# Lennart0HU/Master-Thesis-Deep-Reinforcement-Learning-DDPG-in-Home-Energy-Management

Hardware: AMD Instinct MI355X
Metric: env-steps/sec (higher is better)
Workload: dtype f32; 1 GPU; 65536 parallel shems_LU1 envs per GPU, Charger98 synthetic train table (4320 rows), 72-step episodes, mode=train; envs_per_gpu=65536, episode_len=72, mode=train

## Files before the change

master-thesis-deep-reinforcement-learning-ddpg-in-home-energy-management_amd/_build.py:

```python
from __future__ import annotations

import os
import shutil
import subprocess

HERE = os.path.dirname(os.path.abspath(__file__))
CSRC = os.path.join(HERE, "csrc")
ROOT = os.path.dirname(HERE)
LIB = os.path.join(HERE, "libshems_hip.so")
ARCH = "gfx950"

UNITS = [
    ("shems_capi.hip", []),
    ("shems_env.hip", ["-ffp-contract=off"]),
    ("shems_policy.hip", []),
    ("shems_ddpg.hip", []),
    ("shems_gupd.hip", []),
    ("shems_track.hip", ["-ffp-contract=off"]),
    ("shems_foresight.hip", ["-ffp-contract=off"]),
    ("shems_wide.hip", []),
    ("shems_train.hip", []),
    ("shems_dp.hip", []),
]
COMMON = ["-O3", "-fPIC", "-std=c++17", f"--offload-arch={ARCH}", "-Wall", "-Wno-unused-function", "-Wno-unused-value", "-Wno-unused-result",
          "-I" + os.path.join(ROOT, "include")]


def _hipcc():
    for cand in (os.environ.get("HIPCC"), shutil.which("hipcc"), "/opt/rocm/bin/hipcc"):
        if cand and os.path.exists(cand):
            return cand
    raise RuntimeError("hipcc not found: libshems_hip.so cannot be built (there is no CPU fallback)")


def _deps(src):
    d = [src]
    for f in os.listdir(CSRC):
        if f.endswith(".h"):
            d.append(os.path.join(CSRC, f))
    d.append(os.path.join(ROOT, "include", "shems_hip.h"))
    d.append(os.path.abspath(__file__))
    return d


def build(force=False, verbose=False, defines=(), tag=""):
    hipcc = _hipcc()
    objs = []
    rebuilt = False
    outdir = HERE if not tag else os.path.join(ROOT, "build")
    objdir = CSRC if not tag else outdir
    os.makedirs(outdir, exist_ok=True)
    lib = os.path.join(outdir, f"libshems_hip{tag}.so")
    for name, extra in UNITS:
        src = os.path.join(CSRC, name)
        if not os.path.exists(src):
            continue
        extra = list(extra) + ["-D" + d for d in defines]
        obj = os.path.join(objdir, name.rsplit(".", 1)[0] + tag + ".o")
        stale = force or not os.path.exists(obj) or any(os.path.getmtime(p) > os.path.getmtime(obj) for p in _deps(src))
        if stale:
            cmd = [hipcc, *COMMON, *extra, "-c", src, "-o", obj]
            if verbose:
                print(" ".join(cmd), flush=True)
            subprocess.check_call(cmd)
            rebuilt = True
        objs.append(obj)
    if rebuilt or not os.path.exists(lib):
        cmd = [hipcc, "-shared", "-fPIC", f"--offload-arch={ARCH}", "-o", lib, *objs, "-ldl"]
        if verbose:
            print(" ".join(cmd), flush=True)
        subprocess.check_call(cmd)
    return lib


if __name__ == "__main__":
    import sys
    if "--stamp-act" in sys.argv:
        print(build(force="--force" in sys.argv, verbose=True, defines=("SHEMS_STAMP_ACT",), tag="_stampact"))
    elif "--stamp" in sys.argv:
        print(build(force="--force" in sys.argv, verbose=True, defines=("SHEMS_STAMP",), tag="_stamp"))
    else:
        print(build(force="--force" in sys.argv, verbose=True))
```

master-thesis-deep-reinforcement-learning-ddpg-in-home-energy-management_amd/csrc/shems_policy.hip:

```cpp
#include <hip/hip_runtime.h>

#include <cstdlib>
#include <cstdio>
#include <cstring>
#include <type_traits>

#include "shems_env_dev.h"
#include "shems_internal.h"

namespace shems {

typedef float f32x16 __attribute__((ext_vector_type(16)));
typedef float f32x4 __attribute__((ext_vector_type(4)));
typedef float f32x2 __attribute__((ext_vector_type(2)));
template <int N> struct FVec { typedef float type __attribute__((ext_vector_type(N))); };
template <> struct FVec<1> { typedef float type; };
template <int N> __device__ __forceinline__ float fvec_get(const typename FVec<N>::type &v, int i) { return v[i]; }
template <> __device__ __forceinline__ float fvec_get<1>(const float &v, int) { return v; }

constexpr int kIn = 9, kH1 = SHEMS_L1, kH2 = SHEMS_L2, kOut = 2;

template <int NA> __device__ __forceinline__ int act_col(int nbase, int t, int row) { return nbase + 64 * (t >> 1) + 2 * row + (t & 1); }
template <int NA> __device__ __forceinline__ typename FVec<NA>::type act_load_a(const float *row_at_nbase, int li);
template <> __device__ __forceinline__ FVec<4>::type act_load_a<4>(const float *p, int li)
{
    const f32x2 x = *reinterpret_cast<const f32x2 *>(p + 2 * li), y = *reinterpret_cast<const f32x2 *>(p + 64 + 2 * li);
    return FVec<4>::type{x[0], x[1], y[0], y[1]};
}
constexpr int kKC = 16;
constexpr int kChunks = 16;
constexpr int kW1K = 10, kW1C = 256;
constexpr int kOffB1 = kIn * kH1, kOffW2 = kOffB1 + kH1, kOffB2 = kOffW2 + kH1 * kH2, kOffW3 = kOffB2 + kH2,
              kOffB3 = kOffW3 + kH2 * kOut;
static_assert(kOffB3 + kOut == SHEMS_ACTOR_PARAMS, "actor layout");
static_assert(kW1K == 10 && kIn == 9, "L1_TILE's MFMA chain is written out for 5 k-steps: 9 inputs + the bias row");
constexpr int kH2P = 512;
constexpr int kTailFloats = kH2P + kH2P * kOut + kOut;

struct ActArgs {
    shems_view v;
    shems_act_params p;
    const float *obs;
    int64_t m;
    int64_t m0;
    float *a_out;
    double *rewards;
    float *rewards_f32;
    double *block_reward;
    double *returns_acc;
    shems_replay ring;
    shems_ring_window win;
    int do_step;
    int use_ring;
    int gcount;
    int64_t gstride;
    int64_t genvs;
    const float *w2t;
    int tm_max;
};

template <class T>
__device__ __forceinline__ T *gsh(T *p, int64_t off)
{
    typedef typename std::conditional<std::is_const<T>::value, const char, char>::type B;
    return p ? reinterpret_cast<T *>(reinterpret_cast<B *>(p) + off) : p;
}

constexpr int kFreeChunkFloats = kKC * 128;
constexpr int kPreDw = 16;
constexpr int act_h_rows(int tm) { return tm == 4 ? 128 : 256; }
constexpr bool act_tail_pre(int tm) { return tm <= 2; }
template <int TM, int NW, int RD>
constexpr size_t act_lds_bytes()
{
    return sizeof(float) * ((NW * RD * kFreeChunkFloats + 16) + act_h_rows(TM) * 32 * TM + kW1K * 32 * TM + kW1K * kW1C +
                            (kTailFloats + 2) + 32 * TM * kIn + (act_tail_pre(TM) ? 32 * TM * kPreDw : 0));
}

__device__ __forceinline__ uint32_t lds_addr(const void *p)
{
    return (uint32_t)(uintptr_t)(const __attribute__((address_space(3))) void *)p;
}
template <int IMM>
__device__ __forceinline__ void glds16_asm(const char *sbase, uint32_t voff, uint32_t lds_base)
{
    asm volatile("s_mov_b32 m0, %2\n\ts_nop 0\n\tglobal_load_lds_dwordx4 %0, %1 offset:%3"
                 :: "v"(voff), "s"(sbase), "s"(lds_base), "i"(IMM) : "memory");
}

__device__ __forceinline__ void glds16_asm_piece8(const char *sbase, uint32_t voff, uint32_t lds_base, int q)
{
    switch (q) {
    case 0: glds16_asm<-4096>(sbase, voff, lds_base); break;
    case 1: glds16_asm<-3072>(sbase, voff, lds_base); break;
    case 2: glds16_asm<-2048>(sbase, voff, lds_base); break;
    case 3: glds16_asm<-1024>(sbase, voff, lds_base); break;
    case 4: glds16_asm<0>(sbase, voff, lds_base); break;
    case 5: glds16_asm<1024>(sbase, voff, lds_base); break;
    case 6: glds16_asm<2048>(sbase, voff, lds_base); break;
    default: glds16_asm<3072>(sbase, voff, lds_base); break;
    }
}

__device__ __forceinline__ float2 gauss_pair(uint64_t seed, uint32_t tick, int64_t i)
{
    const u32x4 x = philox4x32_10((uint32_t)i, (uint32_t)((uint64_t)i >> 32), tick, kStreamNoise, (uint32_t)seed,
                                  (uint32_t)(seed >> 32));
    const float u1 = ((float)(x.x >> 8) + 1.0f) * (1.0f / 16777216.0f);
    const float u2 = u01_24(x.y);
    const float r = sqrtf(-2.0f * logf(u1));
    float s, c;
    sincosf(6.28318530717958647692f * u2, &s, &c);
    return make_float2(r * c, r * s);
}

#ifdef SHEMS_STAMP_ACT
#define PSTAMP(i) do { if (threadIdx.x == 0 && blockIdx.x == 0) { reinterpret_cast<unsigned long long *>(A.block_reward)[2*(i)] = __builtin_amdgcn_s_memtime(); reinterpret_cast<unsigned long long *>(A.block_reward)[2*(i)+1] = __builtin_amdgcn_s_memrealtime(); } } while (0)
#else
#define PSTAMP(i)
#endif
#ifdef SHEMS_STAMP_ACT
#define TSTAMP(i) do { asm volatile("s_waitcnt vmcnt(0) lgkmcnt(0)" ::: "memory"); PSTAMP(i); } while (0)
#else
#define TSTAMP(i)
#endif

struct NoiseDraw { uint32_t a, b, c; };
__device__ __forceinline__ NoiseDraw noise_draw(const shems_act_params &p, int64_t i)
{
    NoiseDraw d = {0u, 0u, 0u};
    if (!p.train) return d;
    if (p.noise_kind == SHEMS_NOISE_EPS) {
        const u32x4 x = philox4x32_10((uint32_t)i, (uint32_t)((uint64_t)i >> 32), p.tick, kStreamNoise, (uint32_t)p.seed, (uint32_t)(p.seed >> 32));
        d.a = x.x; d.b = x.y; d.c = x.z;
    } else {
        const float2 z = gauss_pair(p.seed, p.tick, i);
        d.a = __float_as_uint(z.x); d.b = __float_as_uint(z.y);
    }
    return d;
}

struct TailPre {
    Row nx;
    float h_cur;
    int32_t idx, step, ci;
    NoiseDraw nz;
};
__device__ __forceinline__ void tailpre_store(float *lds, const TailPre &t)
{
    f32x4 *q = reinterpret_cast<f32x4 *>(lds);
    q[0] = f32x4{t.nx.h, t.nx.soc_ev, t.nx.d_e, t.nx.g_e};
    q[1] = f32x4{t.nx.p_buy, t.nx.h_cos, t.nx.h_sin, t.nx.season};
    q[2] = f32x4{t.h_cur, __int_as_float(t.idx), __int_as_float(t.step), __int_as_float(t.ci)};
    q[3] = f32x4{__uint_as_float(t.nz.a), __uint_as_float(t.nz.b), __uint_as_float(t.nz.c), 0.0f};
// ... 723 lines not shown
    typedef typename FVec<TM>::type BVec;
    f32x16 acc[2][TM];
#pragma unroll
    for (int a = 0; a < 2; ++a)
#pragma unroll
        for (int r = 0; r < 16; ++r) {
            const float bias = tl[act_col<2>(nbase, a, (r & 3) + 8 * (r >> 2) + 4 * lh)];
#pragma unroll
            for (int b = 0; b < TM; ++b) acc[a][b][r] = bias;
        }
    constexpr int kGKsteps = (kChunks - 1) * (kKC / 2) + (kH1 - (kChunks - 1) * kKC) / 2;
    f32x2 af_[3];
    BVec bf_[3];
#define G_KSTEP(c, ks)                                                                                          \
    do {                                                                                                        \
        const int K_ = 8 * (c) + (ks), K2_ = K_ + 2;                                                            \
        if (K2_ < kGKsteps) {                                                                                   \
            const int c2_ = K2_ >> 3, kr_ = 2 * (K2_ & 7) + lh;                                                 \
            af_[K2_ % 3] = *reinterpret_cast<const f32x2 *>(Wg + (c2_ % RD) * kGChunkFloats + kr_ * 64 + 2 * li); \
            bf_[K2_ % 3] = *reinterpret_cast<const BVec *>(Hc + (c2_ * kKC + kr_) * BM + TM * li);              \
        }                                                                                                       \
        _Pragma("unroll") for (int b = 0; b < TM; ++b)                                                          \
            acc[0][b] = __builtin_amdgcn_mfma_f32_32x32x2f32(af_[K_ % 3][0], fvec_get<TM>(bf_[K_ % 3], b), acc[0][b], 0, 0, 0); \
        _Pragma("unroll") for (int b = 0; b < TM; ++b)                                                          \
            acc[1][b] = __builtin_amdgcn_mfma_f32_32x32x2f32(af_[K_ % 3][1], fvec_get<TM>(bf_[K_ % 3], b), acc[1][b], 0, 0, 0); \
        __builtin_amdgcn_sched_group_barrier(0x008, TM, 0);                                                     \
        __builtin_amdgcn_sched_group_barrier(0x100, 1, 0);                                                      \
        __builtin_amdgcn_sched_group_barrier(0x008, TM, 0);                                                     \
        __builtin_amdgcn_sched_group_barrier(0x100, 1, 0);                                                      \
        __builtin_amdgcn_sched_barrier(0);                                                                      \
        if ((ks) < g_pieces((c) + RD - 1)) { G_PIECE((c) + RD - 1, (ks) < kGPieces ? (ks) : 0); __builtin_amdgcn_sched_barrier(0); } \
    } while (0)
#define G_CHUNK(c, NKS)                                                                                         \
    do {                                                                                                        \
        _Pragma("unroll") for (int ks = 0; ks < ((NKS) < 6 ? (NKS) : 6); ++ks) G_KSTEP(c, ks);                  \
        if ((c) + 1 < kChunks) {                                                                                \
            constexpr int keep_ = g_keep<RD>(c);                                                                \
            asm volatile("s_waitcnt vmcnt(%0)" ::"n"(keep_) : "memory");       \
            __builtin_amdgcn_sched_barrier(0);                                                                  \
        }                                                                                                       \
        _Pragma("unroll") for (int ks = 6; ks < (NKS); ++ks) G_KSTEP(c, ks);                                    \
    } while (0)
    {
        constexpr int keep0_ = g_keep<RD>(-1);
        asm volatile("s_waitcnt vmcnt(%0)" ::"n"(keep0_) : "memory");
        __builtin_amdgcn_sched_barrier(0);
    }
#ifdef SHEMS_STAMP_ACT
    if (lane == 0 && blockIdx.x == 0) reinterpret_cast<unsigned long long *>(A.block_reward)[48 + wave] = __builtin_amdgcn_s_memtime();
#endif
#pragma unroll
    for (int k0 = 0; k0 < 2; ++k0) {
        af_[k0] = *reinterpret_cast<const f32x2 *>(Wg + (2 * k0 + lh) * 64 + 2 * li);
        bf_[k0] = *reinterpret_cast<const BVec *>(Hc + (2 * k0 + lh) * BM + TM * li);
    }
    __builtin_amdgcn_sched_barrier(0);
    G_CHUNK(0, kKC / 2);  GSTAMP(3, blockIdx.x == 0); G_CHUNK(1, kKC / 2);  G_CHUNK(2, kKC / 2);  G_CHUNK(3, kKC / 2);
    G_CHUNK(4, kKC / 2);  G_CHUNK(5, kKC / 2);  G_CHUNK(6, kKC / 2);  G_CHUNK(7, kKC / 2);
    G_CHUNK(8, kKC / 2);  G_CHUNK(9, kKC / 2);  G_CHUNK(10, kKC / 2); G_CHUNK(11, kKC / 2);
    G_CHUNK(12, kKC / 2); G_CHUNK(13, kKC / 2); G_CHUNK(14, kKC / 2);
    GSTAMP(4, blockIdx.x == 0);
    G_CHUNK(15, (kH1 - (kChunks - 1) * kKC) / 2);

    GSTAMP(10, blockIdx.x == 0);
#ifdef SHEMS_STAMP_ACT
    if (lane == 0 && blockIdx.x == 0) reinterpret_cast<unsigned long long *>(A.block_reward)[32 + wave] = __builtin_amdgcn_s_memtime();
#endif
    {
        const float *w3s = tl + kH2P;
        float u0[TM], u1[TM];
#pragma unroll
        for (int t = 0; t < 2; ++t) {
            float o0[TM], o1[TM];
#pragma unroll
            for (int b = 0; b < TM; ++b) { o0[b] = 0.0f; o1[b] = 0.0f; }
#pragma unroll
            for (int r = 0; r < 16; ++r) {
                const int n = act_col<2>(nbase, t, (r & 3) + 8 * (r >> 2) + 4 * lh);
                const float2 w3 = *reinterpret_cast<const float2 *>(w3s + 2 * n);
#pragma unroll
                for (int b = 0; b < TM; ++b) {
                    const float h = fmaxf(acc[t][b][r], 0.0f);
                    o0[b] = fmaf(h, w3.x, o0[b]);
                    o1[b] = fmaf(h, w3.y, o1[b]);
                }
            }
#pragma unroll
            for (int b = 0; b < TM; ++b) {
                u0[b] = t == 0 ? o0[b] : u0[b] + o0[b];
                u1[b] = t == 0 ? o1[b] : u1[b] + o1[b];
            }
        }
#pragma unroll
        for (int b = 0; b < TM; ++b) {
            const float g0 = u0[b] + __shfl_xor(u0[b], 32, 64), g1 = u1[b] + __shfl_xor(u1[b], 32, 64);
            if (lh == 0) *reinterpret_cast<float2 *>(red + (g * BM + TM * li + b) * 2) = make_float2(g0, g1);
        }
    }
    __syncthreads();
    GSTAMP(8, blockIdx.x == 0);

    double reward = 0.0;
    const int64_t i = env0 + tid;
    bool fin = tid < BM && i < A.m;
    float p0 = 0.0f, p1 = 0.0f;
    if (fin) {
        auto half_sum = [&](int hf, int j) {
            return ((red[((4 * hf) * BM + tid) * 2 + j] + red[((4 * hf + 1) * BM + tid) * 2 + j]) + red[((4 * hf + 2) * BM + tid) * 2 + j]) +
                   red[((4 * hf + 3) * BM + tid) * 2 + j];
        };
        float h00, h01, h10, h11;
        if constexpr (NS == 1) {
            h00 = half_sum(0, 0); h01 = half_sum(0, 1); h10 = half_sum(1, 0); h11 = half_sum(1, 1);
        } else {
            float m0 = half_sum(half, 0), m1 = half_sum(half, 1);
            unsigned long long mine = ((unsigned long long)__float_as_uint(m1) << 32) | __float_as_uint(m0);
            if (mine == kSplitEmpty) { mine = 0x7FC000007FC00000ull; m0 = m1 = __uint_as_float(0x7FC00000u); }
            unsigned long long *slot = X.slot + tile * BM + tid;
            const unsigned long long got = __hip_atomic_exchange(slot, mine, __ATOMIC_RELAXED, __HIP_MEMORY_SCOPE_AGENT);
            if (got == kSplitEmpty) fin = false;
            else __hip_atomic_store(slot, kSplitEmpty, __ATOMIC_RELAXED, __HIP_MEMORY_SCOPE_AGENT);
            const float o0 = __uint_as_float((uint32_t)got), o1 = __uint_as_float((uint32_t)(got >> 32));
            h00 = half == 0 ? m0 : o0; h01 = half == 0 ? m1 : o1;
            h10 = half == 0 ? o0 : m0; h11 = half == 0 ? o1 : m1;
        }
        p0 = tl[kH2P + kH2P * kOut + 0] + (h00 + h10);
        p1 = tl[kH2P + kH2P * kOut + 1] + (h01 + h11);
    }
    GSTAMP(9, blockIdx.x == 0);
    GSTAMP(11, tile == 0 && fin);
    if (fin) reward = act_env_tail<HP>(A, i, p0, p1, learner, goff, A.obs == A.v.obs ? xR + tid * kIn : nullptr, xP + tid * kPreDw, hp, gx);
    GSTAMP(12, tile == 0 && fin);
#ifndef SHEMS_STAMP_ACT
    if (NS == 1 && A.block_reward) {
        __syncthreads();
        double *red64 = reinterpret_cast<double *>(Wc);
        const double s = block_sum(reward, red64, NW);
        if (tid == 0) A.block_reward[tile] = s;
    }
#endif
}
template <int TM, int NW, int NS, int RD>
__global__ __launch_bounds__(64 * NW) void k_actg(ActArgs A, ActSplit X) { k_actg_body<TM, NW, NS, RD, 0>(A, X, nullptr); }
template <int TM, int NW, int NS, int RD>
__global__ __launch_bounds__(64 * NW) void k_actg_hp(ActArgs A, ActSplit X, const shems_group_hparams *hp) { k_actg_body<TM, NW, NS, RD, 1>(A, X, hp); }
template <int TM, int NW, int NS, int RD>
__global__ __launch_bounds__(64 * NW) void k_actg_x(ActArgs A, ActSplit X, const shems_group_hparams *hp, GroupX gx) { k_actg_body<TM, NW, NS, RD, 2>(A, X, hp, gx); }

constexpr int k2CR = 4, k2RD = 4, k2CF = k2CR * 128;
constexpr int k2NCH = (kH1 + k2CR - 1) / k2CR;
constexpr int k2_pieces(int ch) { return ch < 0 || ch >= k2NCH ? 0 : ch == k2NCH - 1 ? (kH1 - (k2NCH - 1) * k2CR + 1) / 2 : k2CR / 2; }
constexpr size_t act2_lds_bytes()
{
    return sizeof(float) * (4 * k2RD * k2CF + 16 + 128 * 64 + kW1K * 64 + (kTailFloats + 2) + 64 * kPreDw + 4);
}

__device__ __forceinline__ void k2_piece(const char *sbase, uint32_t voff, uint32_t lds_base, int q)
{
    if (q == 0) glds16_asm<-1024>(sbase, voff, lds_base); else glds16_asm<0>(sbase, voff, lds_base);
}

template <int HP>
__device__ __forceinline__ void k_act2_body(const ActArgs &A, const shems_group_hparams *hp, const GroupX gx = GroupX{nullptr, nullptr})
{
    constexpr int TM = 2, BM = 64, NA = 4, NT_ = 256, HR = 128;
    extern __shared__ __attribute__((aligned(16))) char smem[];
    float *Wc = reinterpret_cast<float *>(smem);
    float *Hc = Wc + 4 * k2RD * k2CF + 16;
    float *xT = Hc + HR * BM;
    float *tl = xT + kW1K * BM;
    float *xP = tl + (kTailFloats + 2);
    const int tid = threadIdx.x;
    const int lane = tid & 63, wave = __builtin_amdgcn_readfirstlane(tid >> 6);
    const int li = lane & 31, lh = lane >> 5;
    int64_t bid = blockIdx.x;
    if (A.gcount > 1 && (gridDim.x & 7) == 0) bid = (int64_t)(blockIdx.x & 7) * (gridDim.x >> 3) + (blockIdx.x >> 3);
    const int64_t env0 = A.m0 + bid * BM;
    const int64_t learner = A.gcount > 1 ? env0 / A.genvs : 0;
    const int64_t goff = learner * A.gstride;
    const float *__restrict__ P = gsh(A.p.actor, goff);
    const float *__restrict__ s_min = gsh(A.p.s_min, goff), *__restrict__ s_max = gsh(A.p.s_max, goff);
    const int nbase = 128 * wave;

    const char *W2g = reinterpret_cast<const char *>(P + kOffW2);
    float *Wf = Wc + wave * (k2RD * k2CF);
    const uint32_t ring_lds = lds_addr(Wf) + 1024;
    const char *wsbase = W2g + wave * 512;
    uint32_t wvoff[2];
#pragma unroll
    for (int q = 0; q < 2; ++q) wvoff[q] = (uint32_t)((lane >> 5) * (kH2 * 4) + (lane & 31) * 16 + q * (2 * kH2 * 4) - (q - 1) * 1024);
#define K2_PIECE(chunk, q) k2_piece(wsbase + (size_t)(chunk) * (k2CR * kH2 * 4), wvoff[q], ring_lds + ((chunk) % k2RD) * (k2CF * 4), (q))
    TailPre tp;
    const bool view = A.do_step != 0, multi = view && A.v.n_cfg > 1;
    {
        const int64_t pe = min(env0 + (tid & (BM - 1)), A.m - 1);
        const int32_t *pidx = view ? A.v.idx : reinterpret_cast<const int32_t *>(P), *pstep = view ? A.v.step : reinterpret_cast<const int32_t *>(P);
        const uint16_t *pci = multi ? A.v.cfg_of_env : reinterpret_cast<const uint16_t *>(P);
        tp.idx = pidx[view ? pe : 0];
        tp.ci = multi ? (int)pci[pe] : 0;
        tp.step = pstep[view ? pe : 0];
    }
    constexpr int kIt = (BM * kIn + NT_ - 1) / NT_;
    float sv[kIt], lo[kIt], hi[kIt], tv[6];
    const int64_t last = A.m * kIn - 1;
#pragma unroll
    for (int it = 0; it < kIt; ++it) {
        const int e = min(it * NT_ + tid, BM * kIn - 1), k = e % kIn;
        sv[it] = A.obs[min(env0 * kIn + e, last)];
        lo[it] = s_min[k];
        hi[it] = s_max[k];
    }
#pragma unroll
    for (int it = 0; it < 6; ++it) tv[it] = P[kOffB2 + min(it * 256 + tid, kH2 + kH2 * kOut + kOut - 1)];
#define K2_L1_LOAD(gbase, a0_, a1_, kA_, kB_)                                                     \
    _Pragma("unroll") for (int s_ = 0; s_ < kW1K / 2; ++s_) {                                     \
        const int j_ = 2 * s_ + lh;                                                               \
        a0_[s_] = P[j_ * kH1 + min(kA_, kH1 - 1)];                                                \
        a1_[s_] = P[j_ * kH1 + min(kB_, kH1 - 1)];                                                \
    }
    const int t0 = wave, t1 = wave + 4;
    const int kA0 = 32 * (t0 >> 1) + li, kB0 = 32 * (t1 >> 1) + li;
    float wa0[kW1K / 2], wb0[kW1K / 2];
    K2_L1_LOAD(0, wa0, wb0, kA0, kB0)
    tp.nz = noise_draw(A.p, env0 + (tid & (BM - 1)));
    f32x4 ra, rb;
    {
        const int32_t *pc = view ? reinterpret_cast<const int32_t *>(A.v.cfgs + tp.ci) : reinterpret_cast<const int32_t *>(P);
        constexpr int o_row0 = offsetof(shems_config, table_row0) / 4, o_nrow = offsetof(shems_config, nrow) / 4;
        const int32_t row0 = pc[o_row0], nrow = pc[o_nrow];
        const float *tp_tables = view ? A.v.tables : P;
        const int64_t tp_row = view ? (int64_t)row0 + max(min(tp.idx + 1, nrow), 2) - 1 : 1;
        const f32x4 *rp = reinterpret_cast<const f32x4 *>(tp_tables + tp_row * SHEMS_NCOL);
        ra = rp[0]; rb = rp[1];
        tp.h_cur = tp_tables[(tp_row - 1) * SHEMS_NCOL];
    }
#pragma unroll
    for (int it = 0; it < kIt; ++it) {
        const int e = it * NT_ + tid, m = e / kIn, k = e - m * kIn;
        const float x = (sv[it] - lo[it]) / ((hi[it] - lo[it]) + 1e-8f);
        if (e < BM * kIn) xT[k * BM + m] = env0 * kIn + e <= last ? x : 0.0f;
    }
    if (tid < BM) xT[kIn * BM + tid] = 1.0f;
    {
#pragma unroll
        for (int it = 0; it < 6; ++it) {
            const int e = it * 256 + tid;
            if (e < kH2) tl[e] = tv[it];
            else if (e < kH2 + kH2 * kOut) tl[kH2P + (e - kH2)] = tv[it];
            else if (e < kH2 + kH2 * kOut + kOut) tl[kH2P + kH2P * kOut + (e - kH2 - kH2 * kOut)] = tv[it];
        }
        if (tid < kH2P - kH2) tl[kH2 + tid] = 0.0f;
        if (tid < (kH2P - kH2) * kOut) tl[kH2P + kH2 * kOut + tid] = 0.0f;
    }
    asm volatile("s_waitcnt lgkmcnt(0)\n\ts_barrier" ::: "memory");
#pragma unroll
    for (int ch = 0; ch < k2RD - 1; ++ch)
#pragma unroll
        for (int q = 0; q < 2; ++q) K2_PIECE(ch, q);

#define K2_L1_PHASE(gbase, a0_, a1_)                                                              \
    do {                                                                                          \
        const int gA_ = (gbase) + (t0 >> 1), bA_ = t0 & 1, gB_ = (gbase) + (t1 >> 1), bB_ = t1 & 1; \
        float c0_[kW1K / 2], c1_[kW1K / 2], z0_[kW1K / 2], z1_[kW1K / 2];                         \
        _Pragma("unroll") for (int s_ = 0; s_ < kW1K / 2; ++s_) {                                 \
            const int j_ = 2 * s_ + lh;                                                           \
            c0_[s_] = xT[j_ * BM + TM * li + bA_];                                                \
            c1_[s_] = xT[j_ * BM + TM * li + bB_];                                                \
            z0_[s_] = 32 * gA_ + li < kH1 ? a0_[s_] : 0.0f;                                       \
            z1_[s_] = 32 * gB_ + li < kH1 ? a1_[s_] : 0.0f;                                       \
        }                                                                                         \
        f32x16 u0_, u1_;                                                                          \
        asm volatile("s_nop 1\n\t"                                                                \
                     "v_mfma_f32_32x32x2_f32 %0, %2, %7, 0\n\t"                                   \
                     "v_mfma_f32_32x32x2_f32 %1, %12, %17, 0\n\t"                                 \
                     "v_mfma_f32_32x32x2_f32 %0, %3, %8, %0\n\t"                                  \
                     "v_mfma_f32_32x32x2_f32 %1, %13, %18, %1\n\t"                                \
                     "v_mfma_f32_32x32x2_f32 %0, %4, %9, %0\n\t"                                  \
                     "v_mfma_f32_32x32x2_f32 %1, %14, %19, %1\n\t"                                \
                     "v_mfma_f32_32x32x2_f32 %0, %5, %10, %0\n\t"                                 \
                     "v_mfma_f32_32x32x2_f32 %1, %15, %20, %1\n\t"                                \
                     "v_mfma_f32_32x32x2_f32 %0, %6, %11, %0\n\t"                                 \
                     "v_mfma_f32_32x32x2_f32 %1, %16, %21, %1\n\t"                                \
                     "s_nop 15\n\ts_nop 7"                                                        \
                     : "=&v"(u0_), "=&v"(u1_)                                                     \
                     : "v"(z0_[0]), "v"(z0_[1]), "v"(z0_[2]), "v"(z0_[3]), "v"(z0_[4]),           \
                       "v"(c0_[0]), "v"(c0_[1]), "v"(c0_[2]), "v"(c0_[3]), "v"(c0_[4]),           \
                       "v"(z1_[0]), "v"(z1_[1]), "v"(z1_[2]), "v"(z1_[3]), "v"(z1_[4]),           \
                       "v"(c1_[0]), "v"(c1_[1]), "v"(c1_[2]), "v"(c1_[3]), "v"(c1_[4]));          \
        float *d0_ = Hc + ((gA_ * 32) % HR) * BM + TM * li + bA_, *d1_ = Hc + ((gB_ * 32) % HR) * BM + TM * li + bB_; \
        _Pragma("unroll") for (int r_ = 0; r_ < 16; ++r_) {                                       \
            d0_[((r_ & 3) + 8 * (r_ >> 2) + 4 * lh) * BM] = fmaxf(u0_[r_], 0.0f);                 \
            d1_[((r_ & 3) + 8 * (r_ >> 2) + 4 * lh) * BM] = fmaxf(u1_[r_], 0.0f);                 \
        }                                                                                         \
    } while (0)
    K2_L1_PHASE(0, wa0, wb0);
    float wa1[kW1K / 2], wb1[kW1K / 2];
    {
        const int kA1 = 128 + kA0, kB1 = 128 + kB0;
        K2_L1_LOAD(4, wa1, wb1, kA1, kB1)
    }
    tp.nx = Row{ra[0], ra[1], ra[2], ra[3], rb[0], rb[1], rb[2], rb[3]};
    tailpre_store(xP + (tid & (BM - 1)) * kPreDw, tp);
    asm volatile("s_waitcnt lgkmcnt(0)\n\ts_barrier" ::: "memory");

    typedef FVec<NA>::type AVec;
    typedef FVec<TM>::type BVec;
    f32x16 acc[NA][TM];
#pragma unroll
    for (int a = 0; a < NA; ++a)
#pragma unroll
        for (int r = 0; r < 16; ++r) {
            const float bias = tl[act_col<NA>(nbase, a, (r & 3) + 8 * (r >> 2) + 4 * lh)];
#pragma unroll
            for (int b = 0; b < TM; ++b) acc[a][b][r] = bias;
        }
    constexpr int kKsteps = kH1 / 2;
    AVec af_[3];
    BVec bf_[3];
#define K2_KSTEP(K)                                                                                             \
    do {                                                                                                        \
        constexpr int K2_ = (K) + 2, c2_ = K2_ >> 1, klim_ = (K) < 64 ? 64 : kKsteps;                           \
        if (K2_ < klim_) {                                                                                      \
            if ((K2_ & 1) == 0) {                                                                               \
                asm volatile("s_waitcnt vmcnt(%0)" ::"n"(k2_pieces(c2_ + 1)) : "memory");                       \
                __builtin_amdgcn_sched_barrier(0);                                                              \
            }                                                                                                   \
            const int kr_ = 2 * (K2_ & 1) + lh;                                                                 \
            af_[K2_ % 3] = act_load_a<NA>(Wf + (c2_ % k2RD) * k2CF + kr_ * 128, li);                            \
            bf_[K2_ % 3] = *reinterpret_cast<const BVec *>(Hc + ((2 * K2_) % HR + lh) * BM + TM * li);          \
        }                                                                                                       \
        _Pragma("unroll") for (int a = 0; a < NA; ++a)                                                          \
            _Pragma("unroll") for (int b = 0; b < TM; ++b)                                                      \
                acc[a][b] = __builtin_amdgcn_mfma_f32_32x32x2f32(fvec_get<NA>(af_[(K) % 3], a), fvec_get<TM>(bf_[(K) % 3], b), acc[a][b], 0, 0, 0); \
        __builtin_amdgcn_sched_group_barrier(0x008, 2, 0);                                                      \
        __builtin_amdgcn_sched_group_barrier(0x100, 1, 0);                                                      \
        __builtin_amdgcn_sched_group_barrier(0x008, 2, 0);                                                      \
        __builtin_amdgcn_sched_group_barrier(0x100, 1, 0);                                                      \
        __builtin_amdgcn_sched_barrier(0);                                                                      \
        if (((K) & 1) < k2_pieces(((K) >> 1) + k2RD - 1)) { K2_PIECE(((K) >> 1) + k2RD - 1, (K) & 1); __builtin_amdgcn_sched_barrier(0); } \
    } while (0)
#define K2_K4(K) K2_KSTEP(K); K2_KSTEP((K) + 1); K2_KSTEP((K) + 2); K2_KSTEP((K) + 3)
#define K2_K16(K) K2_K4(K); K2_K4((K) + 4); K2_K4((K) + 8); K2_K4((K) + 12)
    asm volatile("s_waitcnt vmcnt(%0)" ::"n"(k2_pieces(1) + k2_pieces(2)) : "memory");
    __builtin_amdgcn_sched_barrier(0);
#pragma unroll
    for (int k0 = 0; k0 < 2; ++k0) {
        af_[k0] = act_load_a<NA>(Wf + (2 * k0 + lh) * 128, li);
        bf_[k0] = *reinterpret_cast<const BVec *>(Hc + (2 * k0 + lh) * BM + TM * li);
    }
    __builtin_amdgcn_sched_barrier(0);
    K2_K16(0); K2_K16(16); K2_K16(32); K2_K16(48);
    asm volatile("s_waitcnt lgkmcnt(0)\n\ts_barrier" ::: "memory");
    K2_L1_PHASE(4, wa1, wb1);
    asm volatile("s_waitcnt lgkmcnt(0)\n\ts_barrier" ::: "memory");
    asm volatile("s_waitcnt vmcnt(%0)" ::"n"(k2_pieces(33) + k2_pieces(34)) : "memory");
    __builtin_amdgcn_sched_barrier(0);
#pragma unroll
    for (int k0 = 0; k0 < 2; ++k0) {
        af_[(64 + k0) % 3] = act_load_a<NA>(Wf + ((32 + (k0 >> 1)) % k2RD) * k2CF + (2 * (k0 & 1) + lh) * 128, li);
        bf_[(64 + k0) % 3] = *reinterpret_cast<const BVec *>(Hc + (2 * k0 + lh) * BM + TM * li);
    }
    __builtin_amdgcn_sched_barrier(0);
    K2_K16(64); K2_K16(80); K2_K16(96); K2_K4(112); K2_K4(116); K2_K4(120); K2_KSTEP(124);

    const float *w3s = tl + kH2P;
#pragma unroll
    for (int gl = 0; gl < 2; ++gl) {
        float u0[TM], u1[TM];
#pragma unroll
        for (int t = 0; t < 2; ++t) {
            const int a = 2 * gl + t;
            float o0[TM], o1[TM];
#pragma unroll
            for (int b = 0; b < TM; ++b) { o0[b] = 0.0f; o1[b] = 0.0f; }
#pragma unroll
            for (int r = 0; r < 16; ++r) {
                const int n = act_col<NA>(nbase, a, (r & 3) + 8 * (r >> 2) + 4 * lh);
                const float2 w3 = *reinterpret_cast<const float2 *>(w3s + 2 * n);
#pragma unroll
                for (int b = 0; b < TM; ++b) {
                    const float h = fmaxf(acc[a][b][r], 0.0f);
                    o0[b] = fmaf(h, w3.x, o0[b]);
                    o1[b] = fmaf(h, w3.y, o1[b]);
                }
            }
#pragma unroll
            for (int b = 0; b < TM; ++b) {
                u0[b] = t == 0 ? o0[b] : u0[b] + o0[b];
                u1[b] = t == 0 ? o1[b] : u1[b] + o1[b];
            }
        }
#pragma unroll
        for (int b = 0; b < TM; ++b) {
            const float g0 = u0[b] + __shfl_xor(u0[b], 32, 64), g1 = u1[b] + __shfl_xor(u1[b], 32, 64);
            if (lh == 0) *reinterpret_cast<float2 *>(Wf + gl * (BM * kOut) + (TM * li + b) * 2) = make_float2(g0, g1);
        }
    }
    __syncthreads();
    double reward = 0.0;
    const int64_t i = env0 + tid;
    if (tid < BM && i < A.m) {
        float hs[2][2];
#pragma unroll
        for (int hf = 0; hf < 2; ++hf)
#pragma unroll
            for (int j = 0; j < 2; ++j) {
                const float *r0 = Wc + (2 * hf) * (k2RD * k2CF), *r1 = Wc + (2 * hf + 1) * (k2RD * k2CF);
                hs[hf][j] = ((r0[tid * 2 + j] + r0[BM * kOut + tid * 2 + j]) + r1[tid * 2 + j]) + r1[BM * kOut + tid * 2 + j];
            }
        const float p0 = tl[kH2P + kH2P * kOut + 0] + (hs[0][0] + hs[1][0]), p1 = tl[kH2P + kH2P * kOut + 1] + (hs[0][1] + hs[1][1]);
        reward = act_env_tail<HP>(A, i, p0, p1, learner, goff, nullptr, xP + tid * kPreDw, hp, gx);
    }
#ifndef SHEMS_STAMP_ACT
    if (A.block_reward) {
        __syncthreads();
        double *red64 = reinterpret_cast<double *>(Hc);
        const double s = block_sum(reward, red64, 4);
        if (tid == 0) A.block_reward[bid] = s;
    }
#endif
}
__global__ __launch_bounds__(256, 2) void k_act2(ActArgs A) { k_act2_body<0>(A, nullptr); }
__global__ __launch_bounds__(256, 2) void k_act2_hp(ActArgs A, const shems_group_hparams *hp) { k_act2_body<1>(A, hp); }
__global__ __launch_bounds__(256, 2) void k_act2_x(ActArgs A, const shems_group_hparams *hp, GroupX gx) { k_act2_body<2>(A, hp, gx); }

static int launch_act2(const ActArgs &a, hipStream_t st, const shems_group_hparams *hp = nullptr, const GroupX *gx = nullptr)
{
    constexpr size_t lds = act2_lds_bytes();
    static_assert(lds <= 80 * 1024, "k_act2: two workgroups must fit a CU's 160 KB");
    static std::atomic<uint64_t> optin{0}, optin_hp{0}, optin_x{0};
    const dim3 grid((unsigned)((a.m - a.m0 + 63) / 64));
    if (gx) {
        if (int rc = lds_optin(optin_x, reinterpret_cast<const void *>(&k_act2_x), (int)lds, "hipFuncSetAttribute(k_act2_x)")) return rc;
        hipLaunchKernelGGL(k_act2_x, grid, dim3(256), lds, st, a, hp, *gx);
        return hip_ok(hipGetLastError(), "k_act2_x launch");
    }
    if (hp) {
        if (int rc = lds_optin(optin_hp, reinterpret_cast<const void *>(&k_act2_hp), (int)lds, "hipFuncSetAttribute(k_act2_hp)")) return rc;
        hipLaunchKernelGGL(k_act2_hp, grid, dim3(256), lds, st, a, hp);
        return hip_ok(hipGetLastError(), "k_act2_hp launch");
    }
    if (int rc = lds_optin(optin, reinterpret_cast<const void *>(&k_act2), (int)lds, "hipFuncSetAttribute(k_act2)")) return rc;
    hipLaunchKernelGGL(k_act2, grid, dim3(256), lds, st, a);
    return hip_ok(hipGetLastError(), "k_act2 launch");
}

static int pick_tm(int64_t m, int tm_max = 0)
{
    const int tm = m >= 256 * 128 ? 4 : m >= 256 * 64 ? 2 : 1;
    return tm_max > 0 && tm > tm_max ? tm_max : tm;
}
static int group_tm_max(int64_t envs_per_learner) { return envs_per_learner % 128 == 0 ? 4 : envs_per_learner % 64 == 0 ? 2 : 1; }

template <int TM, int NW, int RD>
static int launch_act(const ActArgs &a, hipStream_t st, const shems_group_hparams *hp = nullptr, const GroupX *gx = nullptr)
{
    constexpr int BM = 32 * TM;
    const size_t lds = act_lds_bytes<TM, NW, RD>();
    static_assert(act_lds_bytes<TM, NW, RD>() <= 160 * 1024, "k_act: LDS image exceeds 160 KB");
    static std::atomic<uint64_t> optin{0}, optin_hp{0}, optin_x{0};
    const unsigned grid = (unsigned)((a.m - a.m0 + BM - 1) / BM);
    if (gx) {
        if (int rc = lds_optin(optin_x, reinterpret_cast<const void *>(&k_act_x<TM, NW, RD>), (int)lds, "hipFuncSetAttribute(k_act_x)")) return rc;
        hipLaunchKernelGGL((k_act_x<TM, NW, RD>), dim3(grid), dim3(64 * NW), lds, st, a, hp, *gx);
        return hip_ok(hipGetLastError(), "k_act_x launch");
    }
    if (hp) {
        if (int rc = lds_optin(optin_hp, reinterpret_cast<const void *>(&k_act_hp<TM, NW, RD>), (int)lds, "hipFuncSetAttribute(k_act_hp)")) return rc;
        hipLaunchKernelGGL((k_act_hp<TM, NW, RD>), dim3(grid), dim3(64 * NW), lds, st, a, hp);
        return hip_ok(hipGetLastError(), "k_act_hp launch");
    }
    if (int rc = lds_optin(optin, reinterpret_cast<const void *>(&k_act<TM, NW, RD>), (int)lds, "hipFuncSetAttribute(k_act)")) return rc;
    hipLaunchKernelGGL((k_act<TM, NW, RD>), dim3(grid), dim3(64 * NW), lds, st, a);
    return hip_ok(hipGetLastError(), "k_act launch");
}

constexpr int kSplitMaxTiles = 512;
static int split_scratch(hipStream_t st, ActSplit *out)
{
    struct Slot { int dev; hipStream_t st; ActSplit x; };
    static Slot slots[32];
    static int nslots = 0;
    static std::atomic_flag lock = ATOMIC_FLAG_INIT;
    int dev = 0;
    if (int rc = hip_ok(hipGetDevice(&dev), "hipGetDevice")) return rc;
    while (lock.test_and_set(std::memory_order_acquire)) {}
    int rc = SHEMS_OK;
    int found = -1;
    for (int i = 0; i < nslots; ++i)
        if (slots[i].dev == dev && slots[i].st == st) { found = i; break; }
    if (found < 0) {
        if (nslots == 32) rc = set_error(SHEMS_ERR_ARG, "k_actg: more than 32 (device, stream) pairs use the column-split form");
        else {
            ActSplit x = {nullptr};
            const size_t bytes = (size_t)kSplitMaxTiles * 64 * sizeof(unsigned long long);
            rc = hip_ok(hipMalloc((void **)&x.slot, bytes), "hipMalloc(split slots)");
            if (!rc) rc = hip_ok(hipMemset(x.slot, 0xFF, bytes), "hipMemset(split slots)");
            if (!rc) { slots[nslots] = Slot{dev, st, x}; found = nslots++; }
        }
    }
    if (!rc) *out = slots[found].x;
    lock.clear(std::memory_order_release);
    return rc;
}

template <int TM, int NW, int NS, int RD>
static int launch_actg(const ActArgs &a, hipStream_t st, const shems_group_hparams *hp = nullptr, const GroupX *gx = nullptr)
{
    constexpr int BM = 32 * TM;
    constexpr size_t lds = actg_lds_bytes<TM, NW, RD>();
    static_assert(lds <= 160 * 1024, "k_actg: LDS image exceeds 160 KB");
    static std::atomic<uint64_t> optin{0}, optin_hp{0}, optin_x{0};
    if (gx) {
        if (int rc = lds_optin(optin_x, reinterpret_cast<const void *>(&k_actg_x<TM, NW, NS, RD>), (int)lds, "hipFuncSetAttribute(k_actg_x)")) return rc;
    } else if (hp) {
        if (int rc = lds_optin(optin_hp, reinterpret_cast<const void *>(&k_actg_hp<TM, NW, NS, RD>), (int)lds, "hipFuncSetAttribute(k_actg_hp)")) return rc;
    } else if (int rc = lds_optin(optin, reinterpret_cast<const void *>(&k_actg<TM, NW, NS, RD>), (int)lds, "hipFuncSetAttribute(k_actg)")) return rc;
    const int64_t tiles = (a.m - a.m0 + BM - 1) / BM;
    ActSplit x = {nullptr};
    if constexpr (NS == 2) {
        if (tiles > kSplitMaxTiles) return set_error(SHEMS_ERR_ARG, "k_actg: %lld env tiles exceed the split form's scratch", (long long)tiles);
        if (split_scratch(st, &x) != SHEMS_OK) {
            return launch_actg<1, 8, 1, RD>(a, st, hp, gx);
        }
    }
    if (gx) {
        hipLaunchKernelGGL((k_actg_x<TM, NW, NS, RD>), dim3((unsigned)(tiles * NS)), dim3(64 * NW), lds, st, a, x, hp, *gx);
        return hip_ok(hipGetLastError(), "k_actg_x launch");
    }
    if (hp) {
        hipLaunchKernelGGL((k_actg_hp<TM, NW, NS, RD>), dim3((unsigned)(tiles * NS)), dim3(64 * NW), lds, st, a, x, hp);
        return hip_ok(hipGetLastError(), "k_actg_hp launch");
    }
    hipLaunchKernelGGL((k_actg<TM, NW, NS, RD>), dim3((unsigned)(tiles * NS)), dim3(64 * NW), lds, st, a, x);
    return hip_ok(hipGetLastError(), "k_actg launch");
}

static int act_form() { static const int f = []() { const char *e = getenv("SHEMS_ACT_FORM"); return e ? atoi(e) : -1; }(); return f; }
enum ActForm { kAct2, kAct442, kAct242, kAct142, kAct143, kActg1422, kActg1423, kActg1813 };
static const char *act_form_name(ActForm f)
{
    static const char *const names[] = {"shems::k_act2", "shems::k_act<4, 4, 2>", "shems::k_act<2, 4, 2>", "shems::k_act<1, 4, 2>",
                                        "shems::k_act<1, 4, 3>", "shems::k_actg<1, 4, 2, 2>", "shems::k_actg<1, 4, 2, 3>",
                                        "shems::k_actg<1, 8, 1, 3>"};
    return names[f];
}
static int act_form_tile_envs(ActForm f)
{
    switch (f) {
    case kAct2: return 64;
    case kAct442: return 128;
    case kAct242: return 64;
    default: return 32;
    }
}

static ActForm pick_act_form(int64_t cnt, int tm_max, int gcount, bool w2t, bool want_sum)
{
    const int form = act_form();
    if (w2t) {
        const int tmt = pick_tm(cnt, tm_max);
        return tmt == 4 ? kAct442 : tmt == 2 ? kAct242 : kAct142;
    }
    if (form < 0 && cnt > 8192 && gcount <= 1) return kAct2;
    if (form == 12 && (tm_max == 0 || tm_max >= 2)) return kAct2;
    const int tm = pick_tm(cnt, tm_max);
    if (tm == 4) return kAct442;
    if (tm == 2) return kAct242;
    if (form == 2) return kAct142;
    if (form == 3) return kAct143;
    const bool split_fits = (cnt + 31) / 32 <= kSplitMaxTiles;
    if ((form == 10 || (form < 0 && cnt > 128 * 32)) && !want_sum && split_fits) return kActg1422;
    if (form == 8 || !split_fits || (form != 9 && (cnt > 128 * 32 || want_sum))) return kActg1813;
    return kActg1423;
}

static int act_tile_envs(int64_t m) { return act_form_tile_envs(pick_act_form(m, 0, 0, false, true)); }

static int dispatch_act(const ActArgs &a, hipStream_t st, const shems_group_hparams *hp = nullptr, const GroupX *gx = nullptr)
{
#ifdef SHEMS_STAMP_ACT
    const bool want_sum = false;
#else
    const bool want_sum = a.block_reward != nullptr;
// ... 298 lines not shown
```

Baseline: 397.5 million env-steps/s.

## Make k_act2 persistent and prefetch next tile's inputs and weights

Turns the actor+env kernel into a persistent loop with a grid capped at two workgroups per CU. Each workgroup walks its tiles and prefetches the next tile's observations, indices, table rows and the first W2 ring chunks plus L1 weights while finishing the current tile's tail. The aim is to hide per-tile prologue latency and cut block launch overhead. It adds register pressure and LDS for normalization bounds, uses compiler-barrier tricks and a disable-machine-licm flag to curb hoisting, and risks load imbalance or spills.

```diff
diff --git a/master-thesis-deep-reinforcement-learning-ddpg-in-home-energy-management_amd/_build.py b/master-thesis-deep-reinforcement-learning-ddpg-in-home-energy-management_amd/_build.py
--- a/master-thesis-deep-reinforcement-learning-ddpg-in-home-energy-management_amd/_build.py
+++ b/master-thesis-deep-reinforcement-learning-ddpg-in-home-energy-management_amd/_build.py
@@ -13,7 +13,7 @@
 UNITS = [
     ("shems_capi.hip", []),
     ("shems_env.hip", ["-ffp-contract=off"]),
-    ("shems_policy.hip", []),
+    ("shems_policy.hip", ["-mllvm", "-disable-machine-licm"]),
     ("shems_ddpg.hip", []),
     ("shems_gupd.hip", []),
     ("shems_track.hip", ["-ffp-contract=off"]),
diff --git a/master-thesis-deep-reinforcement-learning-ddpg-in-home-energy-management_amd/csrc/shems_policy.hip b/master-thesis-deep-reinforcement-learning-ddpg-in-home-energy-management_amd/csrc/shems_policy.hip
--- a/master-thesis-deep-reinforcement-learning-ddpg-in-home-energy-management_amd/csrc/shems_policy.hip
+++ b/master-thesis-deep-reinforcement-learning-ddpg-in-home-energy-management_amd/csrc/shems_policy.hip
@@ -1,5 +1,6 @@
 #include <hip/hip_runtime.h>
 
+#include <algorithm>
 #include <cstdlib>
 #include <cstdio>
 #include <cstring>
@@ -1029,13 +1030,21 @@
 constexpr int k2_pieces(int ch) { return ch < 0 || ch >= k2NCH ? 0 : ch == k2NCH - 1 ? (kH1 - (k2NCH - 1) * k2CR + 1) / 2 : k2CR / 2; }
 constexpr size_t act2_lds_bytes()
 {
-    return sizeof(float) * (4 * k2RD * k2CF + 16 + 128 * 64 + kW1K * 64 + (kTailFloats + 2) + 64 * kPreDw + 4);
+    return sizeof(float) * (4 * k2RD * k2CF + 16 + 128 * 64 + kW1K * 64 + (kTailFloats + 2) + 64 * kPreDw + 32 + 4);
 }
 
 __device__ __forceinline__ void k2_piece(const char *sbase, uint32_t voff, uint32_t lds_base, int q)
 {
     if (q == 0) glds16_asm<-1024>(sbase, voff, lds_base); else glds16_asm<0>(sbase, voff, lds_base);
 }
+
+__device__ __forceinline__ const ActArgs &k2_args_again()
+{
+    uint32_t z = 0;
+    asm volatile("" : "+s"(z));
+    return *(const ActArgs *)((const __attribute__((address_space(4))) char *)__builtin_amdgcn_kernarg_segment_ptr() + z);
+}
+__device__ __forceinline__ int k2_again(int x) { asm volatile("" : "+v"(x)); return x; }
 
 template <int HP>
 __device__ __forceinline__ void k_act2_body(const ActArgs &A, const shems_group_hparams *hp, const GroupX gx = GroupX{nullptr, nullptr})
@@ -1047,12 +1056,14 @@
     float *xT = Hc + HR * BM;
     float *tl = xT + kW1K * BM;
     float *xP = tl + (kTailFloats + 2);
-    const int tid = threadIdx.x;
+    float *nb = xP + BM * kPreDw;
+    const int tid = threadIdx.x, tid0 = tid;
     const int lane = tid & 63, wave = __builtin_amdgcn_readfirstlane(tid >> 6);
     const int li = lane & 31, lh = lane >> 5;
-    int64_t bid = blockIdx.x;
-    if (A.gcount > 1 && (gridDim.x & 7) == 0) bid = (int64_t)(blockIdx.x & 7) * (gridDim.x >> 3) + (blockIdx.x >> 3);
-    const int64_t env0 = A.m0 + bid * BM;
+    const int64_t ntiles = (A.m - A.m0 + BM - 1) / BM;
+    int64_t tile = blockIdx.x;
+    if (A.gcount > 1 && (gridDim.x & 7) == 0) tile = (int64_t)(blockIdx.x & 7) * (gridDim.x >> 3) + (blockIdx.x >> 3);
+    int64_t env0 = A.m0 + tile * BM;
     const int64_t learner = A.gcount > 1 ? env0 / A.genvs : 0;
     const int64_t goff = learner * A.gstride;
     const float *__restrict__ P = gsh(A.p.actor, goff);
@@ -1066,42 +1077,29 @@
     uint32_t wvoff[2];
 #pragma unroll
     for (int q = 0; q < 2; ++q) wvoff[q] = (uint32_t)((lane >> 5) * (kH2 * 4) + (lane & 31) * 16 + q * (2 * kH2 * 4) - (q - 1) * 1024);
-#define K2_PIECE(chunk, q) k2_piece(wsbase + (size_t)(chunk) * (k2CR * kH2 * 4), wvoff[q], ring_lds + ((chunk) % k2RD) * (k2CF * 4), (q))
-    TailPre tp;
+    const char *wst = wsbase;
+    const float *__restrict__ Pt = P;
+#define K2_PIECE(chunk, q) k2_piece(wst + (size_t)(chunk) * (k2CR * kH2 * 4), wvoff[q], ring_lds + ((chunk) % k2RD) * (k2CF * 4), (q))
+#define K2_RING_START()                                                                           \
+    _Pragma("unroll") for (int ch_ = 0; ch_ < k2RD - 1; ++ch_)                                    \
+        _Pragma("unroll") for (int q_ = 0; q_ < 2; ++q_) K2_PIECE(ch_, q_)
+    K2_RING_START();
     const bool view = A.do_step != 0, multi = view && A.v.n_cfg > 1;
-    {
-        const int64_t pe = min(env0 + (tid & (BM - 1)), A.m - 1);
+    constexpr int kIt = (BM * kIn + NT_ - 1) / NT_;
+    const int64_t last = A.m * kIn - 1;
+    struct TileIn { float sv[kIt]; int32_t idx, step, ci; };
+    auto tile_in = [&](const ActArgs &A, int tid, int64_t e0, TileIn &t) {
+        const int64_t pe = min(e0 + (tid & (BM - 1)), A.m - 1);
         const int32_t *pidx = view ? A.v.idx : reinterpret_cast<const int32_t *>(P), *pstep = view ? A.v.step : reinterpret_cast<const int32_t *>(P);
         const uint16_t *pci = multi ? A.v.cfg_of_env : reinterpret_cast<const uint16_t *>(P);
-        tp.idx = pidx[view ? pe : 0];
-        tp.ci = multi ? (int)pci[pe] : 0;
-        tp.step = pstep[view ? pe : 0];
-    }
-    constexpr int kIt = (BM * kIn + NT_ - 1) / NT_;
-    float sv[kIt], lo[kIt], hi[kIt], tv[6];
-    const int64_t last = A.m * kIn - 1;
-#pragma unroll
-    for (int it = 0; it < kIt; ++it) {
-        const int e = min(it * NT_ + tid, BM * kIn - 1), k = e % kIn;
-        sv[it] = A.obs[min(env0 * kIn + e, last)];
-        lo[it] = s_min[k];
-        hi[it] = s_max[k];
-    }
-#pragma unroll
-    for (int it = 0; it < 6; ++it) tv[it] = P[kOffB2 + min(it * 256 + tid, kH2 + kH2 * kOut + kOut - 1)];
-#define K2_L1_LOAD(gbase, a0_, a1_, kA_, kB_)                                                     \
-    _Pragma("unroll") for (int s_ = 0; s_ < kW1K / 2; ++s_) {                                     \
-        const int j_ = 2 * s_ + lh;                                                               \
-        a0_[s_] = P[j_ * kH1 + min(kA_, kH1 - 1)];                                                \
-        a1_[s_] = P[j_ * kH1 + min(kB_, kH1 - 1)];                                                \
-    }
-    const int t0 = wave, t1 = wave + 4;
-    const int kA0 = 32 * (t0 >> 1) + li, kB0 = 32 * (t1 >> 1) + li;
-    float wa0[kW1K / 2], wb0[kW1K / 2];
-    K2_L1_LOAD(0, wa0, wb0, kA0, kB0)
-    tp.nz = noise_draw(A.p, env0 + (tid & (BM - 1)));
-    f32x4 ra, rb;
-    {
+        t.idx = pidx[view ? pe : 0];
+        t.ci = multi ? (int)pci[pe] : 0;
+        t.step = pstep[view ? pe : 0];
+#pragma unroll
+        for (int it = 0; it < kIt; ++it) t.sv[it] = A.obs[min(e0 * kIn + min(it * NT_ + tid, BM * kIn - 1), last)];
+    };
+    auto tile_pre = [&](const ActArgs &A, int tid, int64_t e0, const TileIn &t, TailPre &tp, f32x4 &ra, f32x4 &rb) {
+        tp.idx = t.idx; tp.ci = t.ci; tp.step = t.step;
         const int32_t *pc = view ? reinterpret_cast<const int32_t *>(A.v.cfgs + tp.ci) : reinterpret_cast<const int32_t *>(P);
         constexpr int o_row0 = offsetof(shems_config, table_row0) / 4, o_nrow = offsetof(shems_config, nrow) / 4;
         const int32_t row0 = pc[o_row0], nrow = pc[o_nrow];
@@ -1110,14 +1108,27 @@
         const f32x4 *rp = reinterpret_cast<const f32x4 *>(tp_tables + tp_row * SHEMS_NCOL);
         ra = rp[0]; rb = rp[1];
         tp.h_cur = tp_tables[(tp_row - 1) * SHEMS_NCOL];
-    }
-#pragma unroll
-    for (int it = 0; it < kIt; ++it) {
-        const int e = it * NT_ + tid, m = e / kIn, k = e - m * kIn;
-        const float x = (sv[it] - lo[it]) / ((hi[it] - lo[it]) + 1e-8f);
-        if (e < BM * kIn) xT[k * BM + m] = env0 * kIn + e <= last ? x : 0.0f;
-    }
-    if (tid < BM) xT[kIn * BM + tid] = 1.0f;
+        tp.nz = noise_draw(A.p, e0 + (tid & (BM - 1)));
+    };
+    TileIn cur, nxt;
+    tile_in(A, tid, env0, cur);
+    float tv[6];
+    const float nbv = tid < 16 ? s_min[min(tid, kIn - 1)] : s_max[min(tid & 15, kIn - 1)];
+#pragma unroll
+    for (int it = 0; it < 6; ++it) tv[it] = P[kOffB2 + min(it * 256 + tid, kH2 + kH2 * kOut + kOut - 1)];
+#define K2_L1_LOAD(gbase, a0_, a1_, kA_, kB_)                                                     \
+    _Pragma("unroll") for (int s_ = 0; s_ < kW1K / 2; ++s_) {                                     \
+        const int j_ = 2 * s_ + lh;                                                               \
+        a0_[s_] = Pt[j_ * kH1 + min(kA_, kH1 - 1)];                                               \
+        a1_[s_] = Pt[j_ * kH1 + min(kB_, kH1 - 1)];                                               \
+    }
+    const int t0 = wave, t1 = wave + 4;
+    const int kA0 = 32 * (t0 >> 1) + li, kB0 = 32 * (t1 >> 1) + li;
+    float wa0[kW1K / 2], wb0[kW1K / 2];
+    K2_L1_LOAD(0, wa0, wb0, kA0, kB0)
+    TailPre tp;
+    f32x4 ra, rb;
+    tile_pre(A, tid, env0, cur, tp, ra, rb);
     {
 #pragma unroll
         for (int it = 0; it < 6; ++it) {
@@ -1128,12 +1139,8 @@
         }
         if (tid < kH2P - kH2) tl[kH2 + tid] = 0.0f;
         if (tid < (kH2P - kH2) * kOut) tl[kH2P + kH2 * kOut + tid] = 0.0f;
-    }
-    asm volatile("s_waitcnt lgkmcnt(0)\n\ts_barrier" ::: "memory");
-#pragma unroll
-    for (int ch = 0; ch < k2RD - 1; ++ch)
-#pragma unroll
-        for (int q = 0; q < 2; ++q) K2_PIECE(ch, q);
+        if (tid < 32) nb[tid] = nbv;
+    }
 
 #define K2_L1_PHASE(gbase, a0_, a1_)                                                              \
     do {                                                                                          \
@@ -1170,27 +1177,54 @@
             d1_[((r_ & 3) + 8 * (r_ >> 2) + 4 * lh) * BM] = fmaxf(u1_[r_], 0.0f);                 \
         }                                                                                         \
     } while (0)
-    K2_L1_PHASE(0, wa0, wb0);
+    for (;;) {
+    const int64_t tile_next = tile + gridDim.x;
+    const bool has_next = tile_next < ntiles;
+    const int64_t env0_next = A.m0 + tile_next * BM;
+    uint32_t zt = 0;
+    asm volatile("" : "+s"(zt));
+    const char *wst = wsbase + zt;
+    const float *__restrict__ Pt = P + zt;
+#define K2_FRESH_LANE const int tid = k2_again(tid0), lane = tid & 63, li = lane & 31, lh = lane >> 5;
+    {
+        K2_FRESH_LANE
+        (void)li; (void)lh;
+#pragma unroll
+        for (int it = 0; it < kIt; ++it) {
+            const int e = it * NT_ + tid, m = e / kIn, k = e - m * kIn;
+            const float lo = nb[min(k, kIn - 1)], hi = nb[16 + min(k, kIn - 1)];
+            const float x = (cur.sv[it] - lo) / ((hi - lo) + 1e-8f);
+            if (e < BM * kIn) xT[k * BM + m] = env0 * kIn + e <= last ? x : 0.0f;
+        }
+        if (tid < BM) xT[kIn * BM + tid] = 1.0f;
+    }
+    asm volatile("s_waitcnt lgkmcnt(0)\n\ts_barrier" ::: "memory");
     float wa1[kW1K / 2], wb1[kW1K / 2];
     {
-        const int kA1 = 128 + kA0, kB1 = 128 + kB0;
+        K2_FRESH_LANE
+        K2_L1_PHASE(0, wa0, wb0);
+        const int kA1 = 128 + 32 * (t0 >> 1) + li, kB1 = 128 + 32 * (t1 >> 1) + li;
         K2_L1_LOAD(4, wa1, wb1, kA1, kB1)
-    }
-    tp.nx = Row{ra[0], ra[1], ra[2], ra[3], rb[0], rb[1], rb[2], rb[3]};
-    tailpre_store(xP + (tid & (BM - 1)) * kPreDw, tp);
+        tp.nx = Row{ra[0], ra[1], ra[2], ra[3], rb[0], rb[1], rb[2], rb[3]};
+        tailpre_store(xP + (tid & (BM - 1)) * kPreDw, tp);
+    }
     asm volatile("s_waitcnt lgkmcnt(0)\n\ts_barrier" ::: "memory");
 
     typedef FVec<NA>::type AVec;
     typedef FVec<TM>::type BVec;
     f32x16 acc[NA][TM];
-#pragma unroll
-    for (int a = 0; a < NA; ++a)
-#pragma unroll
-        for (int r = 0; r < 16; ++r) {
-            const float bias = tl[act_col<NA>(nbase, a, (r & 3) + 8 * (r >> 2) + 4 * lh)];
-#pragma unroll
-            for (int b = 0; b < TM; ++b) acc[a][b][r] = bias;
-        }
+    {
+        K2_FRESH_LANE
+        (void)li;
+#pragma unroll
+        for (int a = 0; a < NA; ++a)
+#pragma unroll
+            for (int r = 0; r < 16; ++r) {
+                const float bias = tl[act_col<NA>(nbase, a, (r & 3) + 8 * (r >> 2) + 4 * lh)];
+#pragma unroll
+                for (int b = 0; b < TM; ++b) acc[a][b][r] = bias;
+            }
+    }
     constexpr int kKsteps = kH1 / 2;
     AVec af_[3];
     BVec bf_[3];
@@ -1228,7 +1262,11 @@
     __builtin_amdgcn_sched_barrier(0);
     K2_K16(0); K2_K16(16); K2_K16(32); K2_K16(48);
     asm volatile("s_waitcnt lgkmcnt(0)\n\ts_barrier" ::: "memory");
-    K2_L1_PHASE(4, wa1, wb1);
+    {
+        K2_FRESH_LANE
+        if (has_next) tile_in(k2_args_again(), tid, env0_next, nxt);
+        K2_L1_PHASE(4, wa1, wb1);
+    }
     asm volatile("s_waitcnt lgkmcnt(0)\n\ts_barrier" ::: "memory");
     asm volatile("s_waitcnt vmcnt(%0)" ::"n"(k2_pieces(33) + k2_pieces(34)) : "memory");
     __builtin_amdgcn_sched_barrier(0);
@@ -1240,6 +1278,18 @@
     __builtin_amdgcn_sched_barrier(0);
     K2_K16(64); K2_K16(80); K2_K16(96); K2_K4(112); K2_K4(116); K2_K4(120); K2_KSTEP(124);
 
+    if (has_next) {
+        K2_RING_START();
+        K2_FRESH_LANE
+        (void)tid;
+        const int kA0n = 32 * (t0 >> 1) + li, kB0n = 32 * (t1 >> 1) + li;
+        K2_L1_LOAD(0, wa0, wb0, kA0n, kB0n)
+    }
+
+    {
+    K2_FRESH_LANE
+    (void)tid;
+    float *Ws = Wf + (k2RD - 1) * k2CF;
     const float *w3s = tl + kH2P;
 #pragma unroll
     for (int gl = 0; gl < 2; ++gl) {
@@ -1270,43 +1320,80 @@
 #pragma unroll
         for (int b = 0; b < TM; ++b) {
             const float g0 = u0[b] + __shfl_xor(u0[b], 32, 64), g1 = u1[b] + __shfl_xor(u1[b], 32, 64);
-            if (lh == 0) *reinterpret_cast<float2 *>(Wf + gl * (BM * kOut) + (TM * li + b) * 2) = make_float2(g0, g1);
-        }
-    }
+            if (lh == 0) *reinterpret_cast<float2 *>(Ws + gl * (BM * kOut) + (TM * li + b) * 2) = make_float2(g0, g1);
+        }
+    }
+    }
+    const ActArgs &At = k2_args_again();
+    const int tt = k2_again(tid0);
+    if (has_next) tile_pre(At, tt, env0_next, nxt, tp, ra, rb);
     __syncthreads();
     double reward = 0.0;
-    const int64_t i = env0 + tid;
-    if (tid < BM && i < A.m) {
+    const int64_t i = env0 + tt;
+    if (tt < BM && i < At.m) {
         float hs[2][2];
 #pragma unroll
         for (int hf = 0; hf < 2; ++hf)
 #pragma unroll
             for (int j = 0; j < 2; ++j) {
-                const float *r0 = Wc + (2 * hf) * (k2RD * k2CF), *r1 = Wc + (2 * hf + 1) * (k2RD * k2CF);
-                hs[hf][j] = ((r0[tid * 2 + j] + r0[BM * kOut + tid * 2 + j]) + r1[tid * 2 + j]) + r1[BM * kOut + tid * 2 + j];
+                const float *r0 = Wc + (2 * hf) * (k2RD * k2CF) + (k2RD - 1) * k2CF, *r1 = r0 + k2RD * k2CF;
+                hs[hf][j] = ((r0[tt * 2 + j] + r0[BM * kOut + tt * 2 + j]) + r1[tt * 2 + j]) + r1[BM * kOut + tt * 2 + j];
             }
         const float p0 = tl[kH2P + kH2P * kOut + 0] + (hs[0][0] + hs[1][0]), p1 = tl[kH2P + kH2P * kOut + 1] + (hs[0][1] + hs[1][1]);
-        reward = act_env_tail<HP>(A, i, p0, p1, learner, goff, nullptr, xP + tid * kPreDw, hp, gx);
+        reward = act_env_tail<HP>(At, i, p0, p1, learner, goff, nullptr, xP + tt * kPreDw, hp, gx);
     }
 #ifndef SHEMS_STAMP_ACT
-    if (A.block_reward) {
+    if (At.block_reward) {
         __syncthreads();
         double *red64 = reinterpret_cast<double *>(Hc);
         const double s = block_sum(reward, red64, 4);
-        if (tid == 0) A.block_reward[bid] = s;
+        if (tt == 0) At.block_reward[tile] = s;
     }
 #endif
+    if (!has_next) break;
+    tile = tile_next;
+    env0 = env0_next;
+    cur = nxt;
+    }
 }
 __global__ __launch_bounds__(256, 2) void k_act2(ActArgs A) { k_act2_body<0>(A, nullptr); }
 __global__ __launch_bounds__(256, 2) void k_act2_hp(ActArgs A, const shems_group_hparams *hp) { k_act2_body<1>(A, hp); }
 __global__ __launch_bounds__(256, 2) void k_act2_x(ActArgs A, const shems_group_hparams *hp, GroupX gx) { k_act2_body<2>(A, hp, gx); }
 
+static int device_cus(int *out)
+{
+    static std::atomic<int> cus[64];
+    int dev = 0;
+    if (int rc = hip_ok(hipGetDevice(&dev), "hipGetDevice")) return rc;
+    std::atomic<int> &slot = cus[dev & 63];
+    int n = slot.load(std::memory_order_acquire);
+    if (n <= 0) {
+        if (int rc = hip_ok(hipDeviceGetAttribute(&n, hipDeviceAttributeMultiprocessorCount, dev), "hipDeviceGetAttribute(multiprocessor count)")) return rc;
+        if (n <= 0) return set_error(SHEMS_ERR_HIP, "device %d reports %d compute units", dev, n);
+        slot.store(n, std::memory_order_release);
+    }
+    *out = n;
+    return SHEMS_OK;
+}
+static int64_t act2_wgs_cap() { static const int64_t n = []() { const char *e = getenv("SHEMS_ACT2_WGS"); return e ? atoll(e) : 0ll; }(); return n; }
+
 static int launch_act2(const ActArgs &a, hipStream_t st, const shems_group_hparams *hp = nullptr, const GroupX *gx = nullptr)
 {
     constexpr size_t lds = act2_lds_bytes();
     static_assert(lds <= 80 * 1024, "k_act2: two workgroups must fit a CU's 160 KB");
     static std::atomic<uint64_t> optin{0}, optin_hp{0}, optin_x{0};
-    const dim3 grid((unsigned)((a.m - a.m0 + 63) / 64));
+    const int64_t tiles = (a.m - a.m0 + 63) / 64;
+    int64_t wgs = tiles;
+    if (a.gcount <= 1) {
+        int64_t cap = act2_wgs_cap();
+        if (cap <= 0) {
+            int cus = 0;
+            if (int rc = device_cus(&cus)) return rc;
+            cap = 2 * (int64_t)cus;
+        }
+        wgs = std::min<int64_t>(tiles, cap);
+    }
+    const dim3 grid((unsigned)wgs);
     if (gx) {
         if (int rc = lds_optin(optin_x, reinterpret_cast<const void *>(&k_act2_x), (int)lds, "hipFuncSetAttribute(k_act2_x)")) return rc;
         hipLaunchKernelGGL(k_act2_x, grid, dim3(256), lds, st, a, hp, *gx);
```

Measured after the change: 396.3 million env-steps/s. About the same (-0.3%).
